# rabbitmq/ra

Hardware: AMD Instinct MI355X
Metric: append_entries decisions/sec across N Raft groups; achieved HBM GB/s vs peak (higher is better)
Workload: dtype u64

## Files before the change

ra_amd/csrc/rgb_kernels.hip:

```cpp
#include <hip/hip_runtime.h>
#include "rgb_internal.h"

#define UNDEF 0xFFFFFFFFFFFFFFFFull
#define SLOT_NONE4 0xFu

#ifdef RGB_PROFILE
#define RGB_KNOB(dev, bit) (((dev).dbg & (bit)) != 0)
#else
#define RGB_KNOB(dev, bit) false
#endif

#ifndef RGB_TICK_BLOCK
#define RGB_TICK_BLOCK 64
#endif
#ifndef RGB_CLASS_MIN_WAVES
#define RGB_CLASS_MIN_WAVES(N) ((N) <= 5 ? 4 : 3)
#endif
#ifndef RGB_MIN_WAVES
#define RGB_MIN_WAVES(N) 2
#endif

namespace {

__host__ __device__ constexpr bool rgb_lead_class(int c) { return c == 1 || c == 3 || c == 4; }
// ... 201 lines not shown
__device__ __forceinline__ void peer_set(u64 (&a)[8], unsigned &dirty, unsigned p, u64 v) {
#pragma unroll
  for (int i = 0; i < N; ++i)
    if ((unsigned)i == p) { a[i] = v; dirty |= 1u << i; }
}

template <class Lane>
__device__ __forceinline__ unsigned prow_at(const Lane &L, unsigned w) { return (((w >> 1) ^ L.peers_swz) << 1) | (w & 1u); }
template <class Lane>
__device__ __forceinline__ u64 prow_get(const Lane &L, unsigned w) {
  return reinterpret_cast<const u64 *>(L.peers_lds)[prow_at(L, w)];
}
template <class Lane>
__device__ __forceinline__ void prow_set(Lane &L, unsigned w, u64 v) {
  const_cast<u64 *>(reinterpret_cast<const u64 *>(L.peers_lds))[prow_at(L, w)] = v;
  L.pdirty |= 1u << w;
}
template <int N, bool PL, class Lane> __device__ __forceinline__ u64 mi_get(const Lane &L, int i) { return PL ? prow_get(L, PEER_MI(i, N)) : L.pmi[i]; }
template <int N, bool PL, class Lane> __device__ __forceinline__ u64 ni_get(const Lane &L, int i) { return PL ? prow_get(L, PEER_NI(i, N)) : L.pni[i]; }
template <int N, bool PL, class Lane> __device__ __forceinline__ u64 cs_get(const Lane &L, int i) { return PL ? prow_get(L, PEER_CS(i, N)) : L.pcs[i]; }
template <int N, bool PL, class Lane> __device__ __forceinline__ void ni_set(Lane &L, int i, u64 v) {
  if (PL) prow_set(L, PEER_NI(i, N), v); else { L.pni[i] = v; L.dni |= 1u << i; }
}
template <int N, bool PL, class Lane> __device__ __forceinline__ u64 mi_of(const Lane &L, unsigned p) { return PL ? (p < (unsigned)N ? prow_get(L, PEER_MI(p, N)) : 0) : peer_get<N>(L.pmi, p); }
template <int N, bool PL, class Lane> __device__ __forceinline__ u64 ni_of(const Lane &L, unsigned p) { return PL ? (p < (unsigned)N ? prow_get(L, PEER_NI(p, N)) : 0) : peer_get<N>(L.pni, p); }
template <int N, bool PL, class Lane> __device__ __forceinline__ void mi_put(Lane &L, unsigned p, u64 v) {
  if (PL) { if (p < (unsigned)N) prow_set(L, PEER_MI(p, N), v); } else peer_set<N>(L.pmi, L.dmi, p, v);
}
template <int N, bool PL, class Lane> __device__ __forceinline__ void ni_put(Lane &L, unsigned p, u64 v) {
  if (PL) { if (p < (unsigned)N) prow_set(L, PEER_NI(p, N), v); } else peer_set<N>(L.pni, L.dni, p, v);
}

template <class Lane>
__device__ __forceinline__ bool range_nonempty(const Lane &L) { return L.first <= L.li; }

#define RGB_RUNS_LDS 8
template <class Lane>
__device__ __forceinline__ ulonglong2 run_pair(const Lane &L, int k) {
  if (L.runs_lds != nullptr && k < RGB_RUNS_LDS) return L.runs_lds[(unsigned)k ^ L.peers_swz];
  return ldg16(L.coh, reinterpret_cast<const ulonglong2 *>(L.runs) + k);
}
template <class Lane>
__device__ __forceinline__ u64 run_word(const Lane &L, int i) {
#ifdef RGB_PROFILE
  const_cast<Lane &>(L).prof_nloads += 1;
#endif
  if (L.runs_lds != nullptr && i < 2 * RGB_RUNS_LDS) {
    const ulonglong2 v = L.runs_lds[(unsigned)(i >> 1) ^ L.peers_swz];
    return (i & 1) ? v.y : v.x;
  }
  return ldg8(L.coh, L.runs + i);
}

template <class Lane>
__device__ __forceinline__ int run_search(const Lane &L, u64 idx, u64 &term) {
  int k = (int)L.n_runs - 3;
  if (k < 0) return -1;
  if (Lane::walk_cache && L.wc_k >= 0 && L.wc_k <= k && idx >= L.wc_start && idx < L.wc_next) {
    term = L.wc_term;
    return L.wc_k;
  }
  ulonglong2 cur = run_pair(L, k);
  u64 upper = L.prs;
#pragma unroll 1
  for (; k >= 0; --k) {
    const ulonglong2 nxt = run_pair(L, k > 0 ? k - 1 : 0);
#ifdef RGB_PROFILE
    const_cast<Lane &>(L).prof_nloads += 2u;
#endif
    if (idx >= cur.x) {
      term = cur.y;
      if (Lane::walk_cache) {
        Lane &M = const_cast<Lane &>(L);
        M.wc_k = k; M.wc_start = cur.x; M.wc_term = cur.y; M.wc_next = upper;
      }
      return k;
    }
    upper = cur.x;
    cur = nxt;
  }
  return -1;
}

template <class Lane>
__device__ __forceinline__ u64 fetch_term(const Lane &L, u64 idx) {
  if (!(range_nonempty(L) && idx >= L.first && idx <= L.li)) return UNDEF;
  if (idx >= L.lrs) return L.lrt;
#ifdef RGB_PROFILE
  if (L.prof_noprobe) return L.lrt;
#endif
  if (L.n_runs >= 2 && idx >= L.prs) return L.prt;
  u64 term = UNDEF;
  run_search(L, idx, term);
  return term;
}

template <class Lane>
__device__ __forceinline__ u64 srv_fetch_term(const Lane &L, u64 idx) {
  u64 t = fetch_term(L, idx);
  if (t == UNDEF && L.si != UNDEF && L.si == idx) return L.st;
  return t;
}

template <class Walk>
__device__ __forceinline__ bool quorum_term_gate(u64 pk, unsigned n_runs, u64 ct, u64 first, u64 li, u64 lrs, u64 lrt,
                                                 u64 si, u64 st, u64 p, Walk walk) {
  u64 t = UNDEF;
  if (first <= li && p >= first && p <= li) {
    if (p >= lrs) t = lrt;
    else if (pk_get(pk, PK_CANON_SH, 1) && n_runs >= 1u && lrt <= ct) return false;
    else t = walk();
  }
  if (t == UNDEF && si != UNDEF && si == p) t = st;
  return t != UNDEF && t == ct;
}

template <class Lane>
__device__ __forceinline__ int find_run(const Lane &L, u64 idx) {
  if (L.n_runs == 0) return -1;
  if (idx >= L.lrs) return (int)L.n_runs - 1;
#ifdef RGB_PROFILE
  if (L.prof_noprobe) return (int)L.n_runs - 1;
#endif
  if (L.n_runs >= 2 && idx >= L.prs) return (int)L.n_runs - 2;
  u64 term;
  return run_search(L, idx, term);
}


template <class Lane>
__device__ __forceinline__ u64 next_log_index(const Lane &L) {
  if (range_nonempty(L)) return L.li + 1;
  if (L.si != UNDEF) return L.si + 1;
  return 0;
}

enum { HLE_OK = 0, HLE_MISMATCH = 1, HLE_MISSING = 2 };
template <class Lane>
__device__ __forceinline__ int has_log_entry_or_snapshot(const Lane &L, u64 idx, u64 term) {
  u64 t = fetch_term(L, idx);
  if (t == UNDEF) {
    if (L.si != UNDEF && L.si == idx) return L.st == term ? HLE_OK : HLE_MISMATCH;
    return HLE_MISSING;
  }
  return t == term ? HLE_OK : HLE_MISMATCH;
}

template <class Lane>
__device__ __forceinline__ unsigned role_of(const Lane &L) { return (unsigned)pk_get(L.pk, PK_ROLE_SH, 3); }
template <class Lane>
__device__ __forceinline__ unsigned self_of(const Lane &L) { return (unsigned)pk_get(L.pk, PK_SELF_SH, 4); }
template <class Lane>
__device__ __forceinline__ bool present(const Lane &L, unsigned i) {
  return i < 8u && ((L.pk >> (PK_PRESENT_SH + i)) & 1ull);
}
template <class Lane>
__device__ __forceinline__ bool voter(const Lane &L, unsigned i) { return (L.pk >> (PK_VOTER_SH + i)) & 1ull; }
template <class Lane>
__device__ __forceinline__ bool status_normal(const Lane &L, unsigned i) { return (L.pk >> (PK_STATUS_SH + i)) & 1ull; }

template <class Lane>
__device__ __forceinline__ void set_role(Lane &L, unsigned role) {
  unsigned old = role_of(L);
  if (old != role) L.flags |= RGB_F_ROLE_CHANGED;
  if (role == RGB_ROLE_FOLLOWER && old != RGB_ROLE_FOLLOWER) {
    L.pk = pk_set(L.pk, PK_STATUS_SH, 8, 0xFF);
    L.pk = pk_set(L.pk, PK_BACKOFF_SH, 1, 0);
  }
  if (role != RGB_ROLE_AWAIT_CONDITION) L.pk &= ~((3ull << PK_COND_SH) | (1ull << PK_CONDTO_SH));
  L.pk = pk_set(L.pk, PK_ROLE_SH, 3, role);
}

template <class Lane>
__device__ __forceinline__ void update_term_and_voted_for(Lane &L, u64 term, unsigned voted4) {
  unsigned cur = (unsigned)pk_get(L.pk, PK_VOTED_SH, 4);
  if (term == L.ct && voted4 == cur) return;
  L.flags |= RGB_F_PERSIST;
  L.ct = term;
  L.pk = pk_set(L.pk, PK_VOTED_SH, 4, voted4);
  if (pk_get(L.pk, PK_QPEER_SH, 1)) {
    L.pk = pk_set(L.pk, PK_QPEER_SH, 1, 0);
    if (L.q_loaded) {
#pragma unroll
      for (int i = 0; i < 8; ++i) L.qp[i] = 0;
    }
  }
}

template <class Lane>
__device__ __forceinline__ u64 *qry_row(const Lane &L) { return L.qry_base + (size_t)L.server * RGB_QRY_WORDS; }

template <int N, class Lane>
__device__ __forceinline__ void load_qry(Lane &L) {
  if (L.q_loaded) return;
  const ulonglong2 *qp = reinterpret_cast<const ulonglong2 *>(qry_row(L));
  u64 w[N + 2];
#pragma unroll
  for (int k = 0; k < (N + 2) / 2; ++k) { ulonglong2 v = ldg16(L.coh, qp + k); w[2 * k] = v.x; w[2 * k + 1] = v.y; }
  L.qself = w[0];
  if (pk_get(L.pk, PK_QPEER_SH, 1)) {
#pragma unroll
    for (int i = 0; i < N; ++i) L.qp[i] = w[1 + i];
  }
  L.q_loaded = true;
}

template <class Lane>
__device__ __forceinline__ void heartbeat_reply(Lane &L, u64 term, u64 query_index, unsigned to8) {
// ... 91 lines not shown
      n += use[i] ? 1 : 0;
    }
  }
  L.flags |= RGB_F_QUERY_QUORUM;
  L.q_consensus = agreed_commit<N>(v, use, n);
}
template <class Lane>
__device__ __forceinline__ void update_term(Lane &L, u64 term) {
  if (term != UNDEF && term > L.ct) update_term_and_voted_for(L, term, SLOT_NONE4);
}
template <class Lane>
__device__ __forceinline__ void set_leader_id(Lane &L, unsigned l4) {
  if ((unsigned)pk_get(L.pk, PK_LEADER_SH, 4) != l4) L.flags |= RGB_F_LEADER_CHANGED;
  L.pk = pk_set(L.pk, PK_LEADER_SH, 4, l4);
}

template <class Lane>
__device__ __forceinline__ void aer_reply(Lane &L, u64 term, bool success, unsigned to8) {
  L.has_reply = true;
  L.flags |= RGB_F_REPLY | (success ? RGB_F_REPLY_SUCCESS : 0u);
  L.r_term = term; L.r_next = L.li + 1; L.r_last = L.lwi; L.r_lterm = L.lwt;
  L.reply_to = to8;
}
template <class Lane>
__device__ __forceinline__ void vote_reply(Lane &L, u64 term, bool granted, unsigned to8) {
  L.has_reply = true;
  L.flags |= RGB_F_REPLY | RGB_F_REPLY_VOTE | (granted ? RGB_F_REPLY_SUCCESS : 0u);
  L.r_term = term; L.r_next = 0; L.r_last = 0; L.r_lterm = 0;
  L.reply_to = to8;
}

template <class Lane>
__device__ __forceinline__ void pre_vote_reply(Lane &L, u64 term, u64 token, bool granted, unsigned to8) {
  L.has_reply = true;
  L.flags |= RGB_F_REPLY | RGB_F_REPLY_PRE_VOTE | (granted ? RGB_F_REPLY_SUCCESS : 0u);
  L.r_term = term; L.r_next = token; L.r_last = 0; L.r_lterm = 0;
  L.reply_to = to8;
}

template <class Lane>
__device__ __forceinline__ void call_reply(Lane &L, unsigned code, unsigned to8) {
  L.has_reply = true;
  L.flags |= RGB_F_CALL_REPLY;
  L.r_term = 0; L.r_next = code; L.r_last = 0; L.r_lterm = 0;
  L.reply_to = to8;
}

template <class Lane>
__device__ __forceinline__ unsigned required_quorum(const Lane &L) {
  unsigned voters = __popc((unsigned)(pk_get(L.pk, PK_PRESENT_SH, 8) & pk_get(L.pk, PK_VOTER_SH, 8)));
  return voters / 2 + 1;
}

template <class Lane>
__device__ __forceinline__ bool apply_to(Lane &L, u64 upto) {
  if (upto > L.la) {
    u64 to = L.li < upto ? L.li : upto;
    if (to >= L.la + 1) { L.la = to; return true; }
  }
  return false;
}

template <class Lane>
__device__ __forceinline__ void evaluate_commit_index_follower(Lane &L) {
  if (pk_get(L.pk, PK_LEADER_SH, 4) == SLOT_NONE4) return;
  u64 at = L.li < L.ci ? L.li : L.ci;
  if (apply_to(L, at)) L.flags |= RGB_F_APPLIED | RGB_F_AUX_EVAL;
}


template <class Lane>
__device__ __forceinline__ void push_segment(Lane &L, u64 s, u64 t) {
  if (L.n_runs > 0 && L.lrt == t) return;
  if (L.n_runs == 0) L.pk = pk_set(L.pk, PK_CANON_SH, 1, s <= L.first ? 1ull : 0ull);
  else if (t < L.lrt || s <= L.lrs) L.pk &= ~(1ull << PK_CANON_SH);
  L.prs = L.lrs; L.prt = L.lrt;
  L.push_cnt += 1;
  L.n_runs += 1;
  L.lrs = s; L.lrt = t;
}

template <class Lane>
__device__ __forceinline__ void truncate_runs_to(Lane &L, u64 keep_idx) {
  int k = find_run(L, keep_idx);
  if (k < 0) { L.n_runs = 0; return; }
  if ((unsigned)k != L.n_runs - 1) {
    if ((unsigned)k == L.n_runs - 2) { L.lrs = L.prs; L.lrt = L.prt; }
    else { L.lrs = run_word(L, 2 * k); L.lrt = run_word(L, 2 * k + 1); }
    L.n_runs = (unsigned)k + 1;
    if (k >= 1) { L.prs = run_word(L, 2 * k - 2); L.prt = run_word(L, 2 * k - 1); }
  }
}

template <class Lane>
__device__ __forceinline__ bool pend_nonempty(const Lane &L) { return range_nonempty(L) && L.pend <= L.li; }
template <class Lane>
__device__ __forceinline__ void pend_canon(Lane &L) { if (!pend_nonempty(L)) L.pend = L.li + 1; }
template <class Lane>
__device__ __forceinline__ void pend_old_limit(Lane &L, u64 ceil_excl) { if (ceil_excl < L.po_cut) L.po_cut = ceil_excl; }
template <class Lane>
__device__ __forceinline__ void pend_old_floor(Lane &L, u64 floor_incl) { if (floor_incl > L.po_floor) L.po_floor = floor_incl; }

template <class Lane>
__device__ __forceinline__ int log_write(Lane &L, u32 k0) {
  const u64 base = L.a + 1 + (u64)L.gap;
  const u64 fst = base + k0;
  const u64 lst = base + (L.n_entries - 1);
  const bool had_range = range_nonempty(L);
  if (had_range && !(fst <= L.li + 1)) return RGB_INV_WRITE_INTEGRITY;
  if (fst == 0) return RGB_INV_WRITE_INTEGRITY;
  const bool range_lost = had_range && L.first > lst;
  if (range_lost && L.si == UNDEF) return RGB_INV_WRITE_INTEGRITY;
  u64 lwi = fst - 1 < L.lwi ? fst - 1 : L.lwi;
  u64 lwt;
  if (lwi == L.lwi) lwt = L.lwt;
  else if (L.si != UNDEF && L.si == lwi) lwt = L.st;
  else if (lwi == 0) lwt = 0;
  else {
    lwt = fetch_term(L, lwi);
    if (lwt == UNDEF) return RGB_INV_LAST_WRITTEN_TERM;
  }
  if (!had_range) {
    L.first = fst; L.n_runs = 0;
  } else if (fst <= L.li) {
    if (fst == 0 || fst <= L.first) L.n_runs = 0;
    else truncate_runs_to(L, fst - 1);
  }
  const u64 lo = (had_range && L.first > fst) ? L.first : fst;
  if (range_lost) {
    L.n_runs = 0; L.push_cnt = 0;
    L.li = L.si; L.lt = L.st; L.first = L.si + 1;
  } else {
    if (k0 < L.n_run0) {
      const u64 s1 = base + L.n_run0;
      if (L.n_run0 == L.n_entries || lo < s1) push_segment(L, lo, L.run0_term);
      if (L.n_run0 < L.n_entries) push_segment(L, s1 > lo ? s1 : lo, L.run1_term);
    } else {
      push_segment(L, lo, L.run1_term);
    }
    L.li = lst;
    L.lt = (L.n_entries - 1) < L.n_run0 ? L.run0_term : L.run1_term;
  }
  L.lwi = lwi; L.lwt = lwt;
  if (fst < L.pend) L.pend = fst;
  pend_old_limit(L, fst);
  return 0;
}

template <class Lane>
__device__ __forceinline__ int log_set_last_index(Lane &L, u64 idx) {
  u64 t = fetch_term(L, idx);
  bool snap_is_idx = (L.si != UNDEF && L.si == idx);
  if (t == UNDEF && !snap_is_idx) return RGB_INV_SET_LAST_INDEX_NOT_FOUND;
  if (snap_is_idx) {
    if (range_nonempty(L)) {
      if (idx + 1 <= L.first) { L.n_runs = 0; L.li = idx; L.first = idx + 1; }
      else if (idx + 1 <= L.li) { truncate_runs_to(L, idx); L.li = idx; }
    }
    if (!range_nonempty(L)) L.li = L.si;
    L.lt = L.st;
    L.lwi = L.si; L.lwt = L.st;
    if (idx + 1 < L.pend) L.pend = idx + 1;
    pend_old_limit(L, idx + 1);
    pend_canon(L);
    return 0;
  }
  u64 lwi = idx < L.lwi ? idx : L.lwi;
// ... 122 lines not shown
  }
  pend_old_floor(L, c + 1);
  if (first_clause) {
    changed = !(L.lwi == c && L.lwt == term);
    L.lwi = c; L.lwt = term;
  }
  return 0;
}

__device__ __forceinline__ bool pend_range_written(u64 ps, u64 pe, u64 c, bool two, u64 w2s, u64 w2e, u64 from, u64 to) {
  if (ps > pe || ps > c) return true;
  const u64 e = pe < c ? pe : c;
  const u64 te = to < c ? to : c, t2e = w2e < c ? w2e : c;
  if (from <= c && ps >= from && e <= te) return true;
  if (two && w2s <= c && ps >= w2s && e <= t2e) return true;
  return false;
}

template <class Lane>
__device__ __forceinline__ int log_written(Lane &L, u64 term, u64 from, u64 to, bool &changed) {
  if (L.mflags & RGB_MF_SEQX) {
    if (Lane::seqx_ok) return log_written_many(L, term, from, to, changed);
    changed = false;
    L.flags |= RGB_F_UNHANDLED;
    return 0;
  }
  changed = false;
  const bool in_range = range_nonempty(L);
  const bool two = (L.mflags & RGB_MF_SEQ2) != 0;
  const u64 w2s = L.run0_term, w2e = L.run1_term;
  bool have1 = false; u64 c1 = 0;
  bool have2 = false; u64 c2 = 0;
#pragma unroll 1
  for (int r = 0; r < (two ? 2 : 1); ++r) {
    const u64 f = r ? w2s : from, t = r ? w2e : to;
    if (in_range && !have1) have1 = written_c1(L, term, f, t, c1);
    if (!have2) have2 = written_c2(L, in_range, f, t, c2);
  }
  const bool first_clause = have1 && (!have2 || c1 > c2);
  if (!first_clause && !have2) return 0;
  const u64 c = first_clause ? c1 : c2;
  bool prefix = true;
  const bool sparse = pk_get(L.pk, PK_PENDX_SH, 1) != 0;
  if (pend_nonempty(L)) prefix = pend_range_written(L.pend, L.li, c, two, w2s, w2e, from, to);
  if (sparse && prefix) {
    const u64 *q = qry_row(L);
#pragma unroll 1
    for (int k = 0; k < 2 && prefix; ++k) {
      u64 ps = ldg8(L.coh, q + QRY_PEND_LO + 2 * k), pe = ldg8(L.coh, q + QRY_PEND_LO + 2 * k + 1);
      if (ps < L.po_floor) ps = L.po_floor;
      if (L.po_cut != UNDEF && pe >= L.po_cut) pe = L.po_cut - 1;
      if (L.po_cut == 0) continue;
      prefix = pend_range_written(ps, pe, c, two, w2s, w2e, from, to);
    }
  }
  if (!prefix) {
    if (first_clause) { L.flags |= RGB_F_RESEND_PENDING; return 0; }
    return RGB_INV_WRITTEN_NOT_PREFIX;
  }
  if (pend_nonempty(L)) {
    if (c + 1 > L.pend) L.pend = c + 1;
    pend_canon(L);
  }
  pend_old_floor(L, c + 1);
  if (first_clause) {
    changed = !(L.lwi == c && L.lwt == term);
    L.lwi = c; L.lwt = term;
  }
  return 0;
}

template <class Lane>
__device__ __forceinline__ bool log_snapshot_written(Lane &L, u64 idx, u64 term) {
  if (!(range_nonempty(L) && idx >= L.first)) return false;
  bool changed = false;
  if (!(L.lwi > idx)) {
    changed = !(L.lwi == idx && L.lwt == term);
    L.lwi = idx; L.lwt = term;
  }
  if (idx >= L.li) {
    L.li = idx; L.lt = term; L.first = idx + 1; L.n_runs = 0;
  } else {
    const u64 nf = idx + 1;
    const int k = find_run(L, nf);
    u64 *runs = const_cast<u64 *>(L.runs);
    if (k > 0) {
      ulonglong2 *rp = reinterpret_cast<ulonglong2 *>(runs);
      const int n_mem = (int)L.n_runs - 2 - k;
#ifdef RGB_X_DECLINE_HIST
      atomicAdd(const_cast<u64 *>(L.dbg_hist) + 96 + (n_mem < 0 ? 0 : n_mem > 15 ? 15 : n_mem), 1ull);
#endif
#pragma unroll 1
      for (int i = 0; i < n_mem; i += 4) {
        ulonglong2 t0 = make_ulonglong2(0, 0), t1 = t0, t2 = t0, t3 = t0;
        t0 = ldg16(L.coh, rp + k + i);
        if (i + 1 < n_mem) t1 = ldg16(L.coh, rp + k + i + 1);
        if (i + 2 < n_mem) t2 = ldg16(L.coh, rp + k + i + 2);
        if (i + 3 < n_mem) t3 = ldg16(L.coh, rp + k + i + 3);
        ST16(rp + i, t0);
        if (i + 1 < n_mem) ST16(rp + i + 1, t1);
        if (i + 2 < n_mem) ST16(rp + i + 2, t2);
        if (i + 3 < n_mem) ST16(rp + i + 3, t3);
      }
      if ((int)L.n_runs - 2 >= k) ST16(rp + (L.n_runs - 2 - (unsigned)k), make_ulonglong2(L.prs, L.prt));
      ST16(rp + (L.n_runs - 1 - (unsigned)k), make_ulonglong2(L.lrs, L.lrt));
      L.n_runs -= (unsigned)k;
    }
    if (L.n_runs > 0) runs[0] = nf;
    if (L.lrs < nf) L.lrs = nf;
    if (L.n_runs == 2) L.prs = nf;
    L.first = nf;
  }
  L.si = idx; L.st = term;
  if (idx + 1 > L.pend) L.pend = idx + 1;
  pend_old_floor(L, idx + 1);
  pend_canon(L);
  return changed;
}


template <int N>
__device__ __forceinline__ u64 agreed_commit(const u64 (&v)[N], const bool (&use)[N], int n) {
  if (n <= 0) return UNDEF;
  u64 a[N];
#pragma unroll
  for (int i = 0; i < N; ++i) a[i] = use[i] ? v[i] : 0ull;
#pragma unroll
  for (int r = 0; r < N; ++r) {
#pragma unroll
    for (int i = r & 1; i + 1 < N; i += 2) {
      const bool sw = a[i + 1] > a[i];
      const u64 hi = sw ? a[i + 1] : a[i], lo = sw ? a[i] : a[i + 1];
      a[i] = hi; a[i + 1] = lo;
    }
  }
  const int k = n / 2;
  u64 res = a[0];
#pragma unroll
  for (int i = 1; i < N; ++i) res = (k == i) ? a[i] : res;
  return res;
}

template <int N, bool PL = false, class Lane>
__device__ __forceinline__ void evaluate_quorum(Lane &L) {
  u64 v[N + 1];
  bool use[N + 1];
  const unsigned self = self_of(L);
  int n = 1;
  v[N] = L.lwi; use[N] = true;
#pragma unroll
  for (int i = 0; i < N; ++i) {
    bool u = ((unsigned)i != self) && present(L, i) && voter(L, i);
    v[i] = mi_get<N, PL>(L, i); use[i] = u;
    n += u ? 1 : 0;
  }
  const u64 ci0 = L.ci;
  u64 p = agreed_commit<N + 1>(v, use, n);
  if (quorum_term_gate(L.pk, L.n_runs, L.ct, L.first, L.li, L.lrs, L.lrt, L.si, L.st, p,
                       [&]() __attribute__((always_inline)) { return fetch_term(L, p); }))
    L.ci = p;
  if (L.ci > ci0) L.flags |= RGB_F_AUX_EVAL;
  if (apply_to(L, L.ci)) L.flags |= RGB_F_APPLIED;
}

template <int N, bool EMIT, bool PL = false, class Lane>
__device__ __forceinline__ int pipeline_rpcs(Lane &L, bool force, u32 max_pipe, u32 max_batch, bool &more,
                             unsigned &n_out, rgb_rpc *rpcs, u32 slot_base, u32 msg_index) {
  const unsigned self = self_of(L);
  const u64 next_log = next_log_index(L);
  more = false;
  n_out = 0;
#pragma unroll
  for (int i = 0; i < N; ++i) {
    if ((unsigned)i == self || !present(L, i) || !status_normal(L, i)) continue;
    const u64 mi = mi_get<N, PL>(L, i), ni = ni_get<N, PL>(L, i), cis = cs_get<N, PL>(L, i);
    if (!(ni < next_log || cis < L.ci)) continue;
// ... 749 lines not shown
    if ((d.w[2] | d.w[3] | d.w[4] | d.w[5]) != 0ull) return false;
    A = d.w[6]; B = d.w[7];
  } else if ((flags & ~plain) == RGB_F_WROTE && kind == RGB_MSG_AER) {
    const u64 fst = d.w[3], lst = d.w[4], la = d.w[7];
    if ((d.w[2] | d.w[5]) != 0ull || fst > lst || lst - fst > 0xFFFFull || la > lst || lst - la > 0xFFFFull) return false;
    A = lst; B = d.w[6];
    aux = (u32)(lst - fst) | ((u32)(lst - la) << 16);
  } else if ((flags & ~plain) == (RGB_F_REPLY | RGB_F_REPLY_SUCCESS) && (kind == RGB_MSG_AER || kind == RGB_MSG_WRITTEN)) {
    const u64 term = d.w[2], next = d.w[3], last = d.w[4], lterm = d.w[5], ci = d.w[6], la = d.w[7];
    if (next == 0ull) return false;
    A = next - 1ull; B = term;
    const u64 d1 = A - last, d2 = term - lterm, d3 = ci + 512ull - A, d4 = A + 1ull - la;
    if (last > A || d1 > 0xFFull || lterm > term || d2 > 0xFull || ci + 512ull < A || d3 > 0x3FFull || la > A + 1ull ||
        d4 > 0x3FFull)
      return false;
    aux = (u32)d1 | ((u32)d2 << 8) | ((u32)d3 << 12) | ((u32)d4 << 22);
  } else {
    return false;
  }
  d.w[1] = (u64)(flags | RGB_F_COMPACT) | ((u64)aux << 32);
  d.w[2] = A; d.w[3] = B;
  return true;
}

template <int N, int KIND, bool PRE = false, bool TR = false, bool SEQXP = (KIND < 0)>
__device__ __forceinline__ void process_message(const rgb_dev &dev, const ulonglong2 m0, const ulonglong2 m1,
                                                const ulonglong2 m2, const ulonglong2 m3, u32 i,
                                                rgb_rpc *__restrict__ rpcs, u32 rpc_slot_base,
                                                u32 msg_index_base, Dec &out, u64 *t_loaded = nullptr,
                                                const ulonglong2 *pre = nullptr, unsigned swz = 0,
                                                const ulonglong2 *prepeers = nullptr,
                                                const ulonglong2 *preruns = nullptr, ulonglong2 *rpc_stash = nullptr) {
  LaneT<TR, (N >= 6 && KIND == RGB_MSG_AER), SEQXP> L;
  L.rpc_stash = rpc_stash;
  L.wc_k = -1; L.wc_start = L.wc_term = L.wc_next = 0;
  L.server = (u32)(m0.x & 0xFFFFFFFFull);
  const unsigned wire_kind = (unsigned)((m0.x >> 32) & 0xFF);
  L.kind = KIND >= 0 ? (unsigned)KIND : wire_kind;
  L.from = (unsigned)((m0.x >> 40) & 0xFF);
  L.mflags = (unsigned)((m0.x >> 48) & 0xFF);
  L.gap = (unsigned)((m0.x >> 56) & 0xFF);
  L.term = m0.y; L.a = m1.x; L.b = m1.y; L.c = m2.x;
  L.n_entries = (u32)(m2.y & 0xFFFFFFFFull);
  L.n_run0 = (u32)(m2.y >> 32);
  L.run0_term = m3.x; L.run1_term = m3.y;
  if (L.n_run0 > L.n_entries) L.n_run0 = L.n_entries;

  if (L.kind == RGB_MSG_NOP) {
    make_decision(out, L.server, 0, RGB_NONE, 0, 0, 0, 0, 0, 0, 0, 0, 0, 0);
    return;
  }
  if (L.server >= dev.n_servers || wire_kind != L.kind) {
    make_decision(out, L.server, 0xFF, RGB_NONE, 0, wire_kind, RGB_F_UNHANDLED, 0, 0, 0, 0, 0, 0, 0);
    return;
  }
  u64 *hot = dev.hot + (size_t)L.server * RGB_HOT_WORDS;
  const ulonglong2 *hp = reinterpret_cast<const ulonglong2 *>(hot);
  ulonglong2 h0, h1, h2, h3, h4, h5, h6, h7;
  if (RGB_KNOB(dev, 8u)) { h0 = h1 = h2 = h3 = h4 = h5 = h6 = h7 = make_ulonglong2(0, 0); h0.y = 0x1Full << PK_PRESENT_SH; }
  else if (PRE) {
    h0 = pre[HOT_P_TERM ^ swz]; h1 = pre[HOT_P_CI ^ swz]; h2 = pre[HOT_P_LI ^ swz]; h3 = pre[HOT_P_LW ^ swz];
    h4 = pre[HOT_P_SI ^ swz]; h5 = pre[HOT_P_FIRST ^ swz]; h6 = pre[HOT_P_LRT ^ swz]; h7 = pre[HOT_P_PEND ^ swz];
  } else {
    h0 = ldg16(TR, hp + HOT_P_TERM); h1 = ldg16(TR, hp + HOT_P_CI); h2 = ldg16(TR, hp + HOT_P_LI); h3 = ldg16(TR, hp + HOT_P_LW);
    h4 = ldg16(TR, hp + HOT_P_SI); h5 = ldg16(TR, hp + HOT_P_FIRST); h6 = ldg16(TR, hp + HOT_P_LRT); h7 = ldg16(TR, hp + HOT_P_PEND);
  }
#ifdef RGB_PROFILE
  L.prof_noprobe = RGB_KNOB(dev, 32u); L.prof_nloads = 0;
#endif
#ifdef RGB_X_DECLINE_HIST
  L.dbg_hist = dev.dbg_buf;
#endif
  if (decltype(L)::seqx_ok) { L.seqx = dev.seq_ranges; L.n_seqx = dev.n_seq_ranges; } else { L.seqx = nullptr; L.n_seqx = 0; }
  L.qry_base = dev.qry;
  L.q_loaded = false; L.q_dirty = 0; L.hb_mask = 0;
  L.qself = 0; L.hb_term = L.hb_qi = L.q_consensus = 0; L.cancel_mask = 0;
#pragma unroll
  for (int i = 0; i < 8; ++i) L.qp[i] = 0;
  L.runs = dev.runs + (size_t)L.server * dev.max_runs * 2;
  L.peers = dev.peers + (size_t)L.server * dev.peer_stride;
  L.max_runs = dev.max_runs;
  L.peers_loaded = false; L.dmi = L.dni = L.dcs = 0; L.dcs_ci = 0;
  L.peers_lds = prepeers; L.peers_swz = swz; L.pdirty = 0;
  L.runs_lds = preruns;
  constexpr bool PL = !TR && PRE && rgb_class_slice(1, (unsigned)N) == 32u &&
                      (KIND == RGB_MSG_AER_REPLY || KIND == RGB_MSG_APPEND || KIND == RGB_MSG_PIPELINE_RPCS);
  if (!PL && (L.kind == RGB_MSG_AER_REPLY || L.kind == RGB_MSG_APPEND || L.kind == RGB_MSG_PIPELINE_RPCS ||
              L.kind == RGB_MSG_TRANSFER_LEADERSHIP) &&
      !RGB_KNOB(dev, 64u)) {
    load_peers<N>(L);
  }
#ifdef RGB_PROFILE
  if (RGB_KNOB(dev, 64u)) {
#pragma unroll
    for (int i = 0; i < 8; ++i) { L.pmi[i] = 0; L.pni[i] = 1; L.pcs[i] = 0; }
    L.peers_loaded = true;
  }
#endif
  if (t_loaded && RGB_KNOB(dev, 16u)) {
#ifndef RGB_HOST_EMULATION
    asm volatile("s_waitcnt vmcnt(0)" ::"v"(h0.x), "v"(h6.y) : "memory");
#endif
    *t_loaded = wall_clock64();
  }
  L.ct = h0.x; L.pk = h0.y; L.ci = h1.x; L.la = h1.y; L.li = h2.x; L.lt = h2.y; L.lwi = h3.x;
  L.lwt = h3.y; L.si = h4.x; L.st = h4.y; L.first = h5.x; L.lrs = h5.y; L.lrt = h6.x;
  L.prs = h6.y; L.prt = h7.x; L.pend = h7.y; L.vote_reqs = false;
  constexpr bool TM = KIND < 0 || KIND == RGB_MSG_ELECTION_TIMEOUT || KIND == RGB_MSG_PRE_VOTE_RPC ||
                      KIND == RGB_MSG_PRE_VOTE_RESULT;
  u64 token0 = 0;
  L.token = 0; L.macver = 0;
  if (TM && (L.kind == RGB_MSG_ELECTION_TIMEOUT || L.kind == RGB_MSG_PRE_VOTE_RPC || L.kind == RGB_MSG_PRE_VOTE_RESULT)) {
    const ulonglong2 tm = ldg16(TR, reinterpret_cast<const ulonglong2 *>(qry_row(L) + QRY_TOKEN));
    L.token = token0 = tm.x; L.macver = tm.y;
  }
  L.flags = 0; L.inv = 0; L.has_reply = false; L.reply_to = RGB_NONE;
  L.r_term = L.r_next = L.r_last = L.r_lterm = 0; L.w_first = L.w_last = 0;
  L.n_runs = (unsigned)pk_get(L.pk, PK_NRUNS_SH, 5);
  L.push_cnt = 0;
  L.cond_dirty = false; L.cr0 = L.cr1 = L.cr2 = L.cr3 = 0;
  L.po_floor = 0; L.po_cut = UNDEF;

  const unsigned role0 = role_of(L);
  const unsigned pkhi0 = (unsigned)(L.pk >> 56);
  const u64 ci0 = L.ci, la0 = L.la;
  const unsigned n_runs0 = L.n_runs;
  unsigned n_rpcs = 0;
  int rc = 0;
  unsigned role1 = role0;
  bool go = true;
  if (role0 == RGB_ROLE_AWAIT_CONDITION) {
    bool reprocess = false;
    rc = handle_await_condition<N>(L, reprocess, dev.cond + (size_t)L.server * 4);
    go = !rc && reprocess;
    if (go) { L.flags |= RGB_F_REPROCESSED; role1 = role_of(L); }
  }
  if (go && role1 != RGB_ROLE_FOLLOWER) {
    bool reprocess = false;
    switch (role1) {
      case RGB_ROLE_LEADER:          rc = handle_leader<N, PL>(L, reprocess, dev, rpcs,
                                                           (rpc_slot_base + i) * (N > 1 ? N - 1 : 1),
                                                           msg_index_base + i, n_rpcs); break;
      case RGB_ROLE_CANDIDATE:       rc = handle_candidate<N>(L, reprocess); break;
      case RGB_ROLE_PRE_VOTE:        rc = handle_pre_vote<N>(L, reprocess); break;
      default: L.flags |= RGB_F_UNHANDLED; break;
    }
    go = !rc && reprocess;
    if (go) L.flags |= RGB_F_REPROCESSED;
  }
  if (go) rc = handle_follower<N>(L);
#ifdef RGB_PROFILE
  if (t_loaded && RGB_KNOB(dev, 16u)) t_loaded[2] = wall_clock64();
#endif
  if (rc) {
    make_decision(out, L.server, role0, RGB_NONE, 0, L.kind, RGB_F_INVARIANT, (u32)rc, 0, 0, 0, 0, ci0, la0);
    return;
  }

#ifndef RGB_HOST_EMULATION
  __builtin_amdgcn_s_waitcnt(0x0F70);
#endif
  if (RGB_KNOB(dev, 1u)) { L.n_runs = n_runs0; L.push_cnt = 0; L.cond_dirty = false; L.dmi = L.dni = L.dcs = 0; L.dcs_ci = 0; L.pdirty = 0; }
  if (L.n_runs != n_runs0 || L.push_cnt) {
    u64 *runs = const_cast<u64 *>(L.runs);
    unsigned nr = L.n_runs;
    if (nr > L.max_runs) {
      unsigned shift = nr - L.max_runs;
      unsigned in_mem = nr - L.push_cnt;
      for (unsigned k = shift; k < in_mem; ++k) {
        const u64 rs = ldg8(TR, runs + 2 * k), rt = ldg8(TR, runs + 2 * k + 1);
        runs[2 * (k - shift)] = rs;
        runs[2 * (k - shift) + 1] = rt;
      }
      nr = L.max_runs;
      L.flags |= RGB_F_RUNS_OVERFLOW;
      u64 nf;
      if (L.push_cnt >= nr) nf = (L.push_cnt == 2 && nr == 2) ? L.prs : L.lrs;
      else nf = ldg8(TR, runs);
      L.first = nf;
      L.n_runs = nr;
    }
    if (L.push_cnt == 2) { runs[2 * (nr - 2)] = L.prs; runs[2 * (nr - 2) + 1] = L.prt; }
    if (L.push_cnt >= 1) { runs[2 * (nr - 1)] = L.lrs; runs[2 * (nr - 1) + 1] = L.lrt; }
  }
  L.pk = pk_set(L.pk, PK_NRUNS_SH, 5, L.n_runs);
  if (L.cond_dirty) {
    ulonglong2 *cp = reinterpret_cast<ulonglong2 *>(dev.cond + (size_t)L.server * 4);
    ST16(cp, make_ulonglong2(L.cr0, L.cr1));
    ST16(cp + 1, make_ulonglong2(L.cr2, L.cr3));
  }
  const bool q_reset = ((pkhi0 >> (PK_QPEER_SH - 56)) & 1u) && !pk_get(L.pk, PK_QPEER_SH, 1);
  if ((L.q_dirty || q_reset) && !RGB_KNOB(dev, 1u)) {
    u64 *q = qry_row(L);
    if (L.q_dirty & 1u) q[0] = L.qself;
#pragma unroll
    for (int i = 0; i < N; ++i)
      if (q_reset || (L.q_dirty & (2u << i))) q[1 + i] = L.qp[i];
  }
  if (PL) {
    if (L.pdirty | L.dcs_ci) {
#pragma unroll
      for (int w = 0; w < 2 * N; ++w)
        if (L.pdirty & (1u << w)) ST8(L.peers + w, prow_get(L, (unsigned)w));
#pragma unroll
      for (int k = 0; k < N; ++k)
        if (L.dcs_ci & (1u << k)) ST8(L.peers + PEER_CS(k, N), L.ci);
    }
  } else if (L.dmi | L.dni | L.dcs | L.dcs_ci) {
#pragma unroll
    for (int k = 0; k < N; ++k) {
      if (L.dmi & (1u << k)) ST8(L.peers + PEER_MI(k, N), L.pmi[k]);
      if (L.dni & (1u << k)) ST8(L.peers + PEER_NI(k, N), L.pni[k]);
      if (L.dcs & (1u << k)) ST8(L.peers + PEER_CS(k, N), L.pcs[k]);
      else if (L.dcs_ci & (1u << k)) ST8(L.peers + PEER_CS(k, N), L.ci);
// ... 2132 lines not shown
```

Baseline: 14.24 billion.

## Bisect canonical run lists and fast-path snapshot_written handling

Adds a binary search over canonical (monotone) run arrays, used by find_run in truncation and snapshot compaction paths in place of the linear walk. Peels the first four-entry chunk of the run-compaction copy so its loads are issued up front. Adds a specialised early path for SNAPSHOT_WRITTEN messages that skips role handlers and the LDS run preload. This cuts global loads on long run lists and removes dispatch overhead for that message kind, at the cost of more code and a changed control flow for that kind.

Result: faster. 14.43 billion, median of 6 (+1.3%).

```diff
diff --git a/ra_amd/csrc/rgb_kernels.hip b/ra_amd/csrc/rgb_kernels.hip
--- a/ra_amd/csrc/rgb_kernels.hip
+++ b/ra_amd/csrc/rgb_kernels.hip
@@ -307,6 +307,54 @@
   return -1;
 }
 
+template <bool WANT_TERM, class Lane>
+__device__ __forceinline__ int run_search_canonical(const Lane &L, u64 idx, u64 &term) {
+  const int top = (int)L.n_runs - 3;
+  if (top < 0) return -1;
+  if (Lane::walk_cache && L.wc_k >= 0 && L.wc_k <= top && idx >= L.wc_start && idx < L.wc_next) {
+    term = L.wc_term;
+    return L.wc_k;
+  }
+  ulonglong2 lo = run_pair(L, top);
+  const ulonglong2 one = run_pair(L, top > 0 ? 1 : 0);
+#ifdef RGB_PROFILE
+  const_cast<Lane &>(L).prof_nloads += top > 0 ? 4u : 2u;
+#endif
+  u64 upper = L.prs;
+  int k = top;
+  if (idx < lo.x) {
+    if (top == 0) return -1;
+    upper = one.x; k = 0;
+    if (idx >= one.x) {
+      int hi = top;
+      upper = lo.x; lo = one; k = 1;
+#pragma unroll 1
+      while (hi - k > 1) {
+        const int mid = (k + hi) >> 1;
+        const ulonglong2 m = run_pair(L, mid);
+#ifdef RGB_PROFILE
+        const_cast<Lane &>(L).prof_nloads += 2u;
+#endif
+        if (idx >= m.x) { lo = m; k = mid; } else { upper = m.x; hi = mid; }
+      }
+    } else if (WANT_TERM || Lane::walk_cache || idx < L.first) {
+      lo = run_pair(L, 0);
+#ifdef RGB_PROFILE
+      const_cast<Lane &>(L).prof_nloads += 2u;
+#endif
+      if (idx < lo.x) return -1;
+    } else {
+      return 0;
+    }
+  }
+  term = lo.y;
+  if (Lane::walk_cache) {
+    Lane &M = const_cast<Lane &>(L);
+    M.wc_k = k; M.wc_start = lo.x; M.wc_term = lo.y; M.wc_next = upper;
+  }
+  return k;
+}
+
 template <class Lane>
 __device__ __forceinline__ u64 fetch_term(const Lane &L, u64 idx) {
   if (!(range_nonempty(L) && idx >= L.first && idx <= L.li)) return UNDEF;
@@ -340,7 +388,7 @@
   return t != UNDEF && t == ct;
 }
 
-template <class Lane>
+template <bool BISECT = false, class Lane>
 __device__ __forceinline__ int find_run(const Lane &L, u64 idx) {
   if (L.n_runs == 0) return -1;
   if (idx >= L.lrs) return (int)L.n_runs - 1;
@@ -349,6 +397,7 @@
 #endif
   if (L.n_runs >= 2 && idx >= L.prs) return (int)L.n_runs - 2;
   u64 term;
+  if (BISECT && pk_get(L.pk, PK_CANON_SH, 1)) return run_search_canonical<false>(L, idx, term);
   return run_search(L, idx, term);
 }
 
@@ -606,7 +655,7 @@
 
 template <class Lane>
 __device__ __forceinline__ void truncate_runs_to(Lane &L, u64 keep_idx) {
-  int k = find_run(L, keep_idx);
+  int k = find_run<true>(L, keep_idx);
   if (k < 0) { L.n_runs = 0; return; }
   if ((unsigned)k != L.n_runs - 1) {
     if ((unsigned)k == L.n_runs - 2) { L.lrs = L.prs; L.lrt = L.prt; }
@@ -895,7 +944,7 @@
     L.li = idx; L.lt = term; L.first = idx + 1; L.n_runs = 0;
   } else {
     const u64 nf = idx + 1;
-    const int k = find_run(L, nf);
+    const int k = find_run<true>(L, nf);
     u64 *runs = const_cast<u64 *>(L.runs);
     if (k > 0) {
       ulonglong2 *rp = reinterpret_cast<ulonglong2 *>(runs);
@@ -903,8 +952,19 @@
 #ifdef RGB_X_DECLINE_HIST
       atomicAdd(const_cast<u64 *>(L.dbg_hist) + 96 + (n_mem < 0 ? 0 : n_mem > 15 ? 15 : n_mem), 1ull);
 #endif
+      if (n_mem > 0) {
+        const int last = n_mem - 1;
+        const ulonglong2 t0 = ldg16(L.coh, rp + k);
+        const ulonglong2 t1 = ldg16(L.coh, rp + k + (last < 1 ? last : 1));
+        const ulonglong2 t2 = ldg16(L.coh, rp + k + (last < 2 ? last : 2));
+        const ulonglong2 t3 = ldg16(L.coh, rp + k + (last < 3 ? last : 3));
+        ST16(rp, t0);
+        if (last >= 1) ST16(rp + 1, t1);
+        if (last >= 2) ST16(rp + 2, t2);
+        if (last >= 3) ST16(rp + 3, t3);
+      }
 #pragma unroll 1
-      for (int i = 0; i < n_mem; i += 4) {
+      for (int i = 4; i < n_mem; i += 4) {
         ulonglong2 t0 = make_ulonglong2(0, 0), t1 = t0, t2 = t0, t3 = t0;
         t0 = ldg16(L.coh, rp + k + i);
         if (i + 1 < n_mem) t1 = ldg16(L.coh, rp + k + i + 1);
@@ -1820,7 +1880,7 @@
   L.max_runs = dev.max_runs;
   L.peers_loaded = false; L.dmi = L.dni = L.dcs = 0; L.dcs_ci = 0;
   L.peers_lds = prepeers; L.peers_swz = swz; L.pdirty = 0;
-  L.runs_lds = preruns;
+  L.runs_lds = KIND == RGB_MSG_SNAPSHOT_WRITTEN ? nullptr : preruns;
   constexpr bool PL = !TR && PRE && rgb_class_slice(1, (unsigned)N) == 32u &&
                       (KIND == RGB_MSG_AER_REPLY || KIND == RGB_MSG_APPEND || KIND == RGB_MSG_PIPELINE_RPCS);
   if (!PL && (L.kind == RGB_MSG_AER_REPLY || L.kind == RGB_MSG_APPEND || L.kind == RGB_MSG_PIPELINE_RPCS ||
@@ -1867,7 +1927,13 @@
   int rc = 0;
   unsigned role1 = role0;
   bool go = true;
-  if (role0 == RGB_ROLE_AWAIT_CONDITION) {
+  if (KIND == RGB_MSG_SNAPSHOT_WRITTEN) {
+    const bool changed = log_snapshot_written(L, L.a, L.b);
+    const unsigned l4 = (unsigned)pk_get(L.pk, PK_LEADER_SH, 4);
+    if (role0 == RGB_ROLE_FOLLOWER && changed && l4 != SLOT_NONE4) aer_reply(L, L.ct, true, slot4to8(l4));
+    go = false;
+  }
+  if (go && role0 == RGB_ROLE_AWAIT_CONDITION) {
     bool reprocess = false;
     rc = handle_await_condition<N>(L, reprocess, dev.cond + (size_t)L.server * 4);
     go = !rc && reprocess;
```
